# jbirky/alabi

Hardware: AMD Instinct MI355X
Metric: surrogate_mcmc_samples_per_sec (higher is better)
Workload: dtype f64

## Files before the change

alabi_amd/_lib.py:

```python
from __future__ import annotations

import ctypes as C
import os
import subprocess

_HERE = os.path.dirname(os.path.abspath(__file__))
CSRC = os.path.join(_HERE, "csrc")
LIB_PATH = os.path.join(CSRC, "libalabi_hip.so")

OK, NOT_PD, BAD_ARG, HIP_ERROR, NOT_COMPUTED, TIMEOUT = 0, 1, 2, 3, 4, 5
UTILITY_CODES = {"bape": 0, "agp": 1, "jones": 2}
KERNEL_CODES = {"ExpSquaredKernel": 0, "Matern32Kernel": 1, "Matern52Kernel": 2, "RationalQuadraticKernel": 3}
MAX_DIM = 64

_vp, _i, _ll, _d = C.c_void_p, C.c_int, C.c_longlong, C.c_double
_ull = C.c_ulonglong
_pd = C.POINTER(C.c_double)
_pi = C.POINTER(C.c_int)
_pll = C.POINTER(C.c_longlong)

SIGNATURES = {
    "alabi_abi_version": (_i, []),
    "alabi_status_string": (C.c_char_p, [_i]),
    "alabi_last_error": (C.c_char_p, []),
# ... 35 lines not shown
    "alabi_ens_set_logp_affine": (_i, [_vp, _d, _d]),
    "alabi_ens_set_normal_prior": (_i, [_vp, _pd, _pd]),
    "alabi_ens_set_logp_map": (_i, [_vp, _i]),
    "alabi_ens_surrogate": (_i, [_vp, _vp, _i, _vp, _vp]),
    "alabi_ens_propose": (_i, [_vp, _vp, _i, _i, _i, _vp, _vp, _vp]),
    "alabi_ens_accept": (_i, [_vp, _vp, _vp, _i, _i, _vp, _vp, _vp, _vp]),
    "alabi_ens_set_moves": (_i, [_vp, _i, _pi, _pd, _pd, _pd]),
    "alabi_ens_set_stream": (_i, [_vp, _i]),
    "alabi_ens_last_path": (_i, [_vp, _pi]),
    "alabi_ens_stream_variant": (_i, [_vp, _pi]),
    "alabi_ens_pair_stats": (_i, [_vp, _pll, _i]),
    "alabi_ens_pair_stats2": (_i, [_vp, _pll, _i]),
    "alabi_ens_group_plan": (_i, [_vp, _pi]),
    "alabi_ens_lnprob": (_i, [_vp, _vp, _vp, _vp]),
    "alabi_ens_run": (_i, [_vp, _vp, _vp, _ll, _ll, _i, _d, _vp, _vp, _vp, _vp]),
    "alabi_chain_autocorr": (_i, [_vp, _ll, _i, _i, _vp, _vp]),
    "alabi_ens_draw": (_i, [_vp, _ll, _i, _d, _vp]),
    "alabi_ens_half_step": (_i, [_vp, _vp, _vp, _i, _i, _i, _i, _vp, _vp]),
    "alabi_dist_unique_id": (_i, [_vp]),
    "alabi_dist_comm_create": (_i, [_vp, _i, _i, C.POINTER(_vp)]),
    "alabi_dist_comm_create_callback": (_i, [_vp, _vp, _i, _i, C.POINTER(_vp)]),
    "alabi_dist_comm_destroy": (_i, [_vp]),
    "alabi_dist_comm_stats": (_i, [_vp, _pll]),
    "alabi_ens_run_sharded": (_i, [_vp, _vp, _vp, _vp, _ll, _ll, _i, _d, _vp, _vp, _vp, _vp]),
    "alabi_ens_step_lists": (_i, [_vp, _i, _vp, _pi, _vp]),
    "alabi_ens_step_with_randoms": (_i, [_vp, _vp, _vp, _vp, _i, _vp, _vp, _vp, _d, _vp, _vp]),
    "alabi_ens_export_draws": (_i, [_vp, _ll, _d, _vp, _pi, _vp, _vp, _vp, _vp, _vp, _vp]),
    "alabi_ens_export_move_draws": (_i, [_vp, _vp, _vp, _vp, _vp]),
    "alabi_ens_step_with_randoms_de": (_i, [_vp, _vp, _vp, _vp, _i, _vp, _vp, _vp, _vp, _vp, _vp]),
    "alabi_ens_export_snooker_draws": (_i, [_vp, _vp, _vp]),
# ... 101 lines not shown
```

alabi_amd/csrc/api.hip:

```cpp
#include <atomic>
#include <cmath>
#include <cstdlib>
#include <mutex>
#include <new>
#include <vector>

#include "gp_device.hpp"

namespace alabi {
thread_local std::string g_last_error;

static inline hipStream_t as_stream(void* s) { return reinterpret_cast<hipStream_t>(s); }

__global__ void __launch_bounds__(256)
copy_factor_kernel(const double* __restrict__ L, int ld, int N, double* __restrict__ out) {
    size_t e = (size_t)blockIdx.x * 256 + threadIdx.x;
    if (e >= (size_t)N * N) return;
    int r = (int)(e / N), c = (int)(e % N);
    out[e] = (c <= r) ? L[(size_t)r * ld + c] : 0.0;
}

namespace {
struct CachedBuf { void* p; size_t bytes; };
std::mutex g_cache_mu;
// ... 540 lines not shown
    const size_t n = (size_t)e->chunk_cap * WT;
    DrawBuffers& b = e->draws;
    hipError_t err = alloc_draws(b, n);
    if (err == hipSuccess) err = hipMalloc(&e->run_state, 4 * sizeof(long long));
    if (err == hipSuccess) err = hipMalloc(&e->consts, 5 * ALABI_MAX_DIM * sizeof(double));
    {
        int dev = 0, n_cu = 0;
        const char* env = getenv("ALABI_ENS_STREAM");
        if (hipGetDevice(&dev) == hipSuccess &&
            hipDeviceGetAttribute(&n_cu, hipDeviceAttributeMultiprocessorCount, dev) == hipSuccess &&
            n_ensembles <= n_cu && !(env && env[0] == '0')) {
            int G = n_cu / n_ensembles;
            if (G > (W + 1) / 2) G = (W + 1) / 2;
            e->stream_grid = G;
            const size_t hist_words = ((size_t)e->chunk_cap + 1) * WT * (d + 2);
            if (err == hipSuccess) err = hipMalloc(&e->hist, hist_words * sizeof(unsigned long long));
            if (err == hipSuccess) err = hipMalloc(&e->err, sizeof(int));
            e->stream_ok = (err == hipSuccess) ? 1 : 0;
        }
    }
    if (err != hipSuccess) {
        alabi_ens_destroy(e);
        return hip_fail(err, "hipMalloc(ensemble buffers)", __FILE__, __LINE__);
    }
    *out = e;
    return ALABI_OK;
}

int alabi_ens_destroy(alabi_ens* e) {
    if (!e) return ALABI_OK;
    if (e->graph_exec) (void)hipGraphExecDestroy(e->graph_exec);
    free_draws(e->draws);
    free_draws(e->draws2);
    free_move_buffers(e->mv);
    if (e->side_stream) (void)hipStreamDestroy(e->side_stream);
    if (e->ev_free) (void)hipEventDestroy(e->ev_free);
    if (e->ev_drawn) (void)hipEventDestroy(e->ev_drawn);
    if (e->run_state) (void)hipFree(e->run_state);
    if (e->consts) (void)hipFree(e->consts);
    if (e->hist) (void)hipFree(e->hist);
    if (e->part) (void)hipFree(e->part);
    if (e->cand) (void)hipFree(e->cand);
    if (e->err) (void)hipFree(e->err);
    ens_pair_release(e);
    delete e;
    return ALABI_OK;
}

int alabi_ens_set_normal_prior(alabi_ens* e, const double* mean, const double* std) {
    if (!e || !mean || !std) return ALABI_BAD_ARGUMENT;
    e->has_prior = 0; e->prior_const = 0.0;
    for (int k = 0; k < ALABI_MAX_DIM; ++k) { e->prior_mean[k] = 0.0; e->prior_istd[k] = 0.0; }
    for (int k = 0; k < e->d; ++k) {
        if (std::isfinite(mean[k]) && std::isfinite(std[k]) && std[k] > 0.0) {
            e->prior_mean[k] = mean[k];
            e->prior_istd[k] = 1.0 / std[k];
            e->prior_const += -std::log(std[k]) - 0.9189385332046727;
            e->has_prior = 1;
// ... 32 lines not shown
        if (kind[k] == 0) { if (!(p0[k] > 1.0) || !std::isfinite(p0[k])) return ALABI_BAD_ARGUMENT; }
        else if (kind[k] == 1) { if (!std::isfinite(p0[k]) || !std::isfinite(p1[k])) return ALABI_BAD_ARGUMENT; de = true; }
        else if (kind[k] == 2) { if (!std::isfinite(p0[k])) return ALABI_BAD_ARGUMENT; snooker = true; }
        else return ALABI_BAD_ARGUMENT;
        mt.kind[k] = kind[k]; mt.cum[k] = cum[k]; mt.p0[k] = p0[k]; mt.p1[k] = p1[k];
    }
    if (n > 0 && !(prev > 0.0)) return ALABI_BAD_ARGUMENT;
    if (de && e->W < 4) return ALABI_BAD_ARGUMENT;
    if (snooker && e->W < 6) return ALABI_BAD_ARGUMENT;
    if (n > 0) { const int st = ensure_move_buffers(e, snooker); if (st != ALABI_OK) return st; }
    mt.n = n;
    e->moves = mt;
    e->has_de = de || snooker;
    e->has_snooker = snooker;
    e->drawn_n = 0;
    e->settings_gen++;
    if (e->graph_exec) { (void)hipGraphExecDestroy(e->graph_exec); e->graph_exec = nullptr; }
    return ALABI_OK;
}

int alabi_ens_set_stream(alabi_ens* e, int enabled) {
    if (!e) return ALABI_BAD_ARGUMENT;
    if (enabled && !(e->hist && e->err)) return ALABI_BAD_ARGUMENT;
    e->stream_ok = enabled ? 1 : 0;
    e->settings_gen++;
    return ALABI_OK;
}

int alabi_ens_stream_variant(alabi_ens* e, int* variant) {
    if (!e || !variant) return ALABI_BAD_ARGUMENT;
// ... 106 lines not shown
    const int n0 = h.n0, n1 = e->W - n0;
    const size_t WT = (size_t)e->W * e->E;
    for (int t = 0; t < n; ++t) {
        h.rec = offset_draws(e->draws, (size_t)t * WT);
        h.cw2 = e->has_de ? e->mv.cw2 + (size_t)t * WT : nullptr;
        h.cw3 = e->has_snooker ? e->mv.cw3 + (size_t)t * WT : nullptr;
        h.local_t = t; h.part_begin = 0;
        h.split = 0;
        if ((st = launch_ens_half_args(e, h, n0, s)) != ALABI_OK) return st;
        h.split = 1;
        if ((st = launch_ens_half_args(e, h, n1, s)) != ALABI_OK) return st;
    }
    return launch_ens_advance(e, n, s);
}

int alabi_ens_run(alabi_ens* e, double* coords, double* logp, long long step0, long long nsteps, int thin_by,
                  double a, double* chain, double* chain_logp, long long* n_accept, void* stream) {
    if (!e || !coords || !logp || nsteps < 0 || thin_by < 1 || !(a > 1.0)) return ALABI_BAD_ARGUMENT;
    if (!e->gp->computed || !e->gp->has_alpha) return ALABI_NOT_COMPUTED;
    if (nsteps == 0) return ALABI_OK;
    hipStream_t s = as_stream(stream);
    int st;
    if ((st = sync_consts(e, s)) != ALABI_OK) return st;
    e->last_path = 0;
    const char* genv = getenv("ALABI_ENS_GROUP");
    const bool group_off = genv && genv[0] == '0', group_pref = genv && genv[0] == '1';
    const bool can_stream = ens_stream_fits(e);
    const bool crowded = can_stream && e->stream_grid > 0 && ((e->W + 1) / 2 + e->stream_grid - 1) / e->stream_grid >= 4;
    const bool use_group = !e->has_de && e->stream_ok && s != nullptr && !group_off && (group_pref || !can_stream || crowded) && ens_group_fits(e) &&
                           ens_group_buffers(e, s);
    if (!e->has_de && e->stream_ok && s != nullptr && (can_stream || use_group)) {
        e->last_path = use_group ? 3 : 1;
        const int need = (int)(nsteps < e->chunk_cap ? nsteps : e->chunk_cap);
        const int clean_rows = e->hist_clean;
        e->hist_clean = 0;
        const bool use_pair = !use_group && can_stream && ens_pair_ready(e);
        e->last_variant = use_pair ? 1 : 0;
        const size_t WTs = (size_t)e->W * e->E;
        if (use_pair) {
            double* sv = e->pair_save;
            ALABI_HIP_CHECK(hipMemcpyAsync(sv, coords, WTs * e->d * sizeof(double), hipMemcpyDeviceToDevice, s));
            ALABI_HIP_CHECK(hipMemcpyAsync(sv + WTs * e->d, logp, WTs * sizeof(double), hipMemcpyDeviceToDevice, s));
            if (n_accept) ALABI_HIP_CHECK(hipMemcpyAsync(sv + WTs * (e->d + 1), n_accept, WTs * sizeof(long long), hipMemcpyDeviceToDevice, s));
        }
        if (use_group && (st = set_run_state(e, step0, 0, s)) != ALABI_OK) return st;
        ALABI_HIP_CHECK(hipMemsetAsync(e->err, 0, sizeof(int), s));
        long long remaining = nsteps;
        const bool two_sets = !use_group && nsteps > e->chunk_cap && ens_draw_ahead_ready(e);
        bool ahead_issued = false;
        while (remaining > 0) {
            const int K = (int)(remaining < e->chunk_cap ? remaining : e->chunk_cap);
            const long long done = nsteps - remaining;
            if (use_group) {
                if ((st = launch_ens_draw(e, K, a, s)) != ALABI_OK) return st;
                if ((st = launch_ens_group(e, coords, logp, K, thin_by, chain, chain_logp, n_accept, s)) != ALABI_OK) return st;
                if ((st = launch_ens_advance(e, K, s)) != ALABI_OK) return st;
            } else {
                const bool odd = two_sets && ((done / e->chunk_cap) & 1);
                const bool ahead = two_sets && remaining > K;
                const DrawBuffers& cur = odd ? e->draws2 : e->draws;
                if (ahead_issued) ALABI_HIP_CHECK(hipStreamWaitEvent(s, e->ev_drawn, 0));
                else if ((st = launch_ens_draw_at(e, cur, K, a, false, step0 + done, s)) != ALABI_OK) return st;
                ahead_issued = false;
                if (ahead) ALABI_HIP_CHECK(hipEventRecord(e->ev_free, s));
                const int fill_rows = (done == 0 && clean_rows < need) ? need : 0;
                if ((st = use_pair ? launch_ens_pair_kernel(e, cur, coords, logp, K, done == 0, fill_rows, s)
                                   : launch_ens_stream_kernel(e, cur, coords, logp, K, done == 0, fill_rows, s)) != ALABI_OK)
                    return st;
                if (ahead) {
                    const long long rem2 = remaining - K;
                    const int K2 = (int)(rem2 < e->chunk_cap ? rem2 : e->chunk_cap);
                    ALABI_HIP_CHECK(hipStreamWaitEvent(e->side_stream, e->ev_free, 0));
                    if ((st = launch_ens_draw_at(e, odd ? e->draws : e->draws2, K2, a, false, step0 + done + K, e->side_stream)) != ALABI_OK)
                        return st;
                    ALABI_HIP_CHECK(hipEventRecord(e->ev_drawn, e->side_stream));
                    ahead_issued = true;
                }
                if ((st = launch_ens_stream_epilogue(e, coords, logp, K, thin_by, chain, chain_logp, n_accept, step0 + done + K, done, s)) != ALABI_OK)
                    return st;
            }
            remaining -= K;
        }
        int flag = 0;
        ALABI_HIP_CHECK(hipMemcpyAsync(&flag, e->err, sizeof(int), hipMemcpyDeviceToHost, s));
        ALABI_HIP_CHECK(hipStreamSynchronize(s));
        e->hist_clean = (!use_group && !flag) ? (clean_rows > need ? clean_rows : need) : 0;
        if (flag && use_pair) {
            const double* sv = e->pair_save;
            ALABI_HIP_CHECK(hipMemcpyAsync(coords, sv, WTs * e->d * sizeof(double), hipMemcpyDeviceToDevice, s));
            ALABI_HIP_CHECK(hipMemcpyAsync(logp, sv + WTs * e->d, WTs * sizeof(double), hipMemcpyDeviceToDevice, s));
            if (n_accept) ALABI_HIP_CHECK(hipMemcpyAsync(n_accept, sv + WTs * (e->d + 1), WTs * sizeof(long long), hipMemcpyDeviceToDevice, s));
            e->pair_state = -1;
            return alabi_ens_run(e, coords, logp, step0, nsteps, thin_by, a, chain, chain_logp, n_accept, stream);
        }
        return flag ? ALABI_TIMEOUT : ALABI_OK;
    }
    if ((st = set_run_state(e, step0, 0, s)) != ALABI_OK) return st;
    HalfArgs h = base_args(e, coords, logp);
    h.chain = chain; h.chain_logp = chain_logp; h.n_accept = n_accept; h.thin_by = thin_by;

    const char* env = getenv("ALABI_ENS_GRAPH");
    const bool want_graph = (s != nullptr) && !(env && env[0] == '0');
    int gsteps = e->chunk_cap < 256 ? e->chunk_cap : 256;
    if (const char* gs = getenv("ALABI_ENS_GRAPH_STEPS")) {
        int v = atoi(gs);
        if (v > 0 && v <= e->chunk_cap) gsteps = v;
// ... 210 lines not shown
```

alabi_amd/csrc/common.hpp:

```cpp
#pragma once
#include <hip/hip_runtime.h>
#include <cstdint>
#include <cstdio>
#include <cstring>
#include <string>
#include <vector>

#include "../../include/alabi_hip.h"
#include "chol_tasks.hpp"

#define ALABI_BLK 64

namespace alabi {

extern thread_local std::string g_last_error;

inline int hip_fail(hipError_t e, const char* what, const char* file, int line) {
    char buf[512];
    snprintf(buf, sizeof(buf), "%s failed at %s:%d: %s", what, file, line, hipGetErrorString(e));
    g_last_error = buf;
    return ALABI_HIP_ERROR;
}

#define ALABI_HIP_CHECK(expr)                                                    \
// ... 116 lines not shown
    long long consts_gen = -1;
    int chunk_cap = 0;
    int drawn_n = 0;
    alabi::DrawBuffers draws{};
    hipGraphExec_t graph_exec = nullptr;
    struct GraphKey {
        void *coords, *logp, *chain, *chain_logp, *n_accept;
        int thin_by, nsteps;
        double a;
        long long gp_gen;
    } graph_key{};
    int graph_steps = 0;
    long long* run_state = nullptr;
    unsigned long long* hist = nullptr;
    int* err = nullptr;
    alabi::DrawBuffers draws2{};
    hipStream_t side_stream = nullptr;
    hipEvent_t ev_free = nullptr, ev_drawn = nullptr;
    int draws2_state = 0;
    int hist_clean = 0;
    int stream_grid = 0;
    int last_path = 0;
    int stream_ok = 0;
    unsigned long long* prop = nullptr;
    double* pair_save = nullptr;
#define ALABI_PAIR_STATS_WORDS 16
    unsigned long long* pair_stats = nullptr;
    int pair_state = 0;
    int last_variant = 0;
    unsigned long long* part = nullptr;
    size_t part_words = 0;
    unsigned long long* cand = nullptr;
    size_t cand_words = 0;
    long long settings_gen = 0;
    long long serial = 0;
    int group_plan[8] = {0};
    alabi::MoveTable moves{};
    bool has_de = false, has_snooker = false;
    alabi::MoveBuffers mv{};
};
// ... 78 lines not shown
                    const double* u_acc, double a, hipStream_t s);
int launch_ens_prep_de(alabi_ens* e, const int* order, int n0, const int* j1, const int* j2, const double* gamma,
                       const double* u_acc, hipStream_t s);
int launch_ens_prep_snooker(alabi_ens* e, const int* order, int n0, const int* j1, const int* j2, const int* j3, double gamma,
                            const double* u_acc, hipStream_t s);
int launch_ens_half_args(alabi_ens* e, const HalfArgs& args, int nblocks, hipStream_t s);
int launch_ens_lnprob(alabi_ens* e, const double* coords, int nwalkers, double* logp, int gate_box, hipStream_t s);
int launch_ens_propose(alabi_ens* e, const HalfArgs& args, int nblocks, int gate_box, double* q, double* like, hipStream_t s);
int launch_ens_accept(alabi_ens* e, const HalfArgs& args, int count, const double* q, const double* lp_new, hipStream_t s);
int launch_ens_advance(alabi_ens* e, long long n, hipStream_t s);
int ens_sync_consts(alabi_ens* e, hipStream_t s);
int alabi_ens_half_step_hist(alabi_ens* e, const double* coords, const double* logp, int t, int split, int part_begin, int part_end,
                             const double* shist, double* out, hipStream_t s);
bool ens_stream_fits(const alabi_ens* e);
int ens_stream_ppt(const alabi_ens* e);
int launch_ens_stream_kernel(alabi_ens* e, const DrawBuffers& rec, double* coords, double* logp, int K, bool first, int fill_rows, hipStream_t s);
int launch_ens_hist_fill(unsigned long long* rows, size_t words, hipStream_t s);
int launch_ens_stream_prologue(alabi_ens* e, double* coords, double* logp, bool first, int fill_rows, hipStream_t s);
int launch_ens_stream_epilogue(alabi_ens* e, double* coords, double* logp, int K, int thin_by, double* chain, double* chain_logp,
                               long long* n_accept, long long step_next, long long done0, hipStream_t s);
int launch_ens_hist_prologue(alabi_ens* e, double* coords, double* logp, int K, bool fill, hipStream_t s);
int launch_ens_hist_epilogue(alabi_ens* e, double* coords, double* logp, int K, int thin_by, double* chain, double* chain_logp,
                             long long* n_accept, hipStream_t s);
bool ens_pair_ready(alabi_ens* e);
void ens_pair_release(alabi_ens* e);
int launch_ens_pair_kernel(alabi_ens* e, const DrawBuffers& rec, double* coords, double* logp, int K, bool first, int fill_rows, hipStream_t s);
bool ens_group_fits(const alabi_ens* e);
bool ens_group_buffers(alabi_ens* e, hipStream_t s);
int launch_ens_group(alabi_ens* e, double* coords, double* logp, int K, int thin_by, double* chain, double* chain_logp,
                     long long* n_accept, hipStream_t s);
}
```

alabi_amd/csrc/ens_pair.hip:

```cpp
#include <cstdlib>
#include "ens_stream.hpp"

namespace alabi {

struct PairArgs {
    StreamArgs s;
    unsigned long long* prop;
    unsigned long long* stats;
};

#ifdef ALABI_PAIR_PROF
__device__ long long g_pair_prof[26];
#define ALABI_PAIR_PUB_MASK ((1 << 19) - 1)
__device__ long long g_pair_pub[2][ALABI_PAIR_PUB_MASK + 1];
__device__ inline void pair_pub_stamp(int which, size_t row_index) {
    __hip_atomic_store(&g_pair_pub[which][row_index & ALABI_PAIR_PUB_MASK], wall_clock64(), __ATOMIC_RELAXED, __HIP_MEMORY_SCOPE_AGENT);
}
__device__ inline long long pair_pub_age(int which, size_t row_index, long long now) {
    const long long dt = now - __hip_atomic_load(&g_pair_pub[which][row_index & ALABI_PAIR_PUB_MASK], __ATOMIC_RELAXED, __HIP_MEMORY_SCOPE_AGENT);
    return (dt > 0 && dt < 100000) ? dt : -1;
}
#endif

template <int D, int PPT, int TMAX, bool GENERIC>
// ... 257 lines not shown
#endif

bool ens_pair_ready(alabi_ens* e) {
    if (e->pair_state < 0) return false;
    if (e->pair_state == 0) {
        e->pair_state = -1;
        const char* env = getenv("ALABI_ENS_PAIR");
        if (env && env[0] == '0') return false;
        int dev = 0, n_cu = 0;
        if (hipGetDevice(&dev) != hipSuccess || hipDeviceGetAttribute(&n_cu, hipDeviceAttributeMultiprocessorCount, dev) != hipSuccess) return false;
        const long long wgs = 2LL * ((e->W + 1) / 2) * e->E;
        if (e->d < 1 || wgs > n_cu) return false;
        const size_t WT = (size_t)e->W * e->E, row = e->d + 2;
        const size_t words = ((size_t)e->chunk_cap + 1) * WT * row;
        if (hipMalloc(&e->prop, words * sizeof(unsigned long long)) != hipSuccess) { (void)hipGetLastError(); e->prop = nullptr; return false; }
        if (hipMalloc(&e->pair_save, (WT * (e->d + 1)) * sizeof(double) + WT * sizeof(long long)) != hipSuccess) {
            (void)hipGetLastError(); (void)hipFree(e->prop); e->prop = nullptr; e->pair_save = nullptr; return false;
        }
        e->pair_state = 1;
    }
    return true;
}

void ens_pair_release(alabi_ens* e) {
    if (e->prop) (void)hipFree(e->prop);
    if (e->pair_save) (void)hipFree(e->pair_save);
    if (e->pair_stats) (void)hipFree(e->pair_stats);
    e->prop = nullptr; e->pair_save = nullptr; e->pair_stats = nullptr;
}

int launch_ens_pair_kernel(alabi_ens* e, const DrawBuffers& rec, double* coords, double* logp, int K, bool first, int fill_rows,
                           hipStream_t s) {
    const int n0 = (e->W + 1) / 2;
    const int WT = e->W * e->E, row = e->d + 2;
    int st = launch_ens_stream_prologue(e, coords, logp, first, fill_rows, s);
    if (st != ALABI_OK) return st;
    if ((st = launch_ens_hist_fill(e->prop + (size_t)WT * row, (size_t)K * WT * row, s)) != ALABI_OK) return st;
    PairArgs a{};
    a.s = ens_stream_args(e, rec, K);
    a.prop = e->prop; a.stats = e->pair_stats;
    e->last_path = 1;
    st = ens_stream_dispatch(e, [&](auto D, auto PPT, auto TMAX, auto GENERIC) {
        hipLaunchKernelGGL((ens_pair_kernel<D(), PPT(), TMAX(), GENERIC()>), dim3(2 * n0, e->E), dim3(TMAX()), 0, s, a);
    });
    if (st != ALABI_OK) return st;
    ALABI_LAUNCH_CHECK();
    return ALABI_OK;
}

}
```

alabi_amd/csrc/ens_stream.hip:

```cpp
#include <cstdlib>
#include "ens_stream.hpp"

namespace alabi {

#ifdef ALABI_STREAM_PROF
__device__ long long g_stream_prof[16];
#endif

template <int D, int PPT, int TMAX, bool GENERIC>
__global__ void __launch_bounds__(TMAX)
ens_stream_kernel(StreamArgs p) {
    __shared__ __attribute__((aligned(16))) double scratch[2][16];
    __shared__ unsigned long long rec_s[4][4];
    __shared__ __attribute__((aligned(16))) double qs_s[2][ALABI_MAX_DIM];
    __shared__ double consts_s[6][ALABI_MAX_DIM];
    __shared__ int abort_s;
    static_assert(D < ALABI_MAX_DIM && TMAX >= 192 && TMAX % 64 == 0, "ens_stream_kernel: shape");
    constexpr int TC = TMAX - 128, nwc = TC >> 6;
    const int tid = threadIdx.x, lane = tid & 63;
    const int wv = __builtin_amdgcn_readfirstlane(tid >> 6);
    const bool comm = wv == 0, service = wv == nwc + 1, compute = !comm && !service;
    const int b = blockIdx.x, e = blockIdx.y, E = gridDim.y;
    const int WT = p.W * E, row = p.d + 2;
#ifdef ALABI_STREAM_PROF
// ... 133 lines not shown
}

__global__ void __launch_bounds__(256)
ens_hist_copy_kernel(double* __restrict__ coords, double* __restrict__ logp, unsigned long long* __restrict__ hist_row,
                     int WT, int d, int to_hist) {
    const int i = blockIdx.x * 256 + threadIdx.x, row = d + 2;
    if (i >= WT * row) return;
    const int w = i / row, k = i % row;
    if (k > d) { if (to_hist) hist_row[i] = 0ull; return; }
    double* src = (k < d) ? coords + (size_t)w * d + k : logp + w;
    if (to_hist) hist_row[i] = (unsigned long long)__double_as_longlong(*src);
    else *src = __longlong_as_double((long long)hist_row[i]);
}

__global__ void __launch_bounds__(256)
ens_hist_chain_kernel(const unsigned long long* __restrict__ hist, int K, int WT, int d, int thin_by,
                      const long long* __restrict__ run_state, const int* __restrict__ err, double* __restrict__ chain,
                      double* __restrict__ chain_logp, unsigned long long* __restrict__ n_accept) {
    if (*err) return;
    const int row = d + 2;
    const size_t n = (size_t)K * WT * row;
    const long long done0 = run_state[1];
    for (size_t i = (size_t)blockIdx.x * 256 + threadIdx.x; i < n; i += (size_t)gridDim.x * 256) {
        const int k = (int)(i % row);
        const size_t vw = i / row;
        const int w = (int)(vw % WT), v = (int)(vw / WT) + 1;
        const unsigned long long word = hist[(size_t)WT * row + i];
        if (k == d + 1) { if (word == 1ull && n_accept) atomicAdd(n_accept + w, 1ull); continue; }
        const long long done = done0 + v;
        if (done % thin_by != 0) continue;
        const size_t slot = (size_t)(done / thin_by - 1);
        if (k < d) { if (chain) chain[(slot * WT + w) * d + k] = __longlong_as_double((long long)word); }
        else if (chain_logp) chain_logp[slot * WT + w] = __longlong_as_double((long long)word);
    }
}

#define ALABI_EPI_VG 16
__global__ void __launch_bounds__(256)
ens_hist_epilogue_kernel(unsigned long long* __restrict__ hist, int K, int WT, int d, int thin_by, long long step_next, long long done0,
                         const int* __restrict__ err, double* __restrict__ coords, double* __restrict__ logp, double* __restrict__ chain,
                         double* __restrict__ chain_logp, unsigned long long* __restrict__ n_accept, long long* __restrict__ run_state) {
    const int k = threadIdx.x, row = d + 2;
    const int w = blockIdx.x * blockDim.y + threadIdx.y;
    if (blockIdx.x == 0 && blockIdx.y == 0 && threadIdx.x == 0 && threadIdx.y == 0) { run_state[0] = step_next; run_state[1] = done0 + K; }
    if (*err) return;
    if (k >= row || w >= WT) return;
    const int v0 = 1 + blockIdx.y * ALABI_EPI_VG;
    const int v1 = (v0 + ALABI_EPI_VG - 1 < K) ? v0 + ALABI_EPI_VG - 1 : K;
    long long slot = (done0 + v0) / thin_by;
    int phase = (int)((done0 + v0) % thin_by);
    const size_t vstride = (size_t)WT * row;
    unsigned long long* hp = hist + (size_t)v0 * vstride + (size_t)w * row + k;
    unsigned long long nacc = 0;
    for (int v = v0; v <= v1; v += 4, hp += 4 * vstride) {
        unsigned long long word[4];
#pragma unroll
        for (int j = 0; j < 4; ++j) word[j] = (v + j <= v1) ? hp[j * vstride] : 0ull;
#pragma unroll
        for (int j = 0; j < 4; ++j) {
            if (v + j > v1) break;
            hp[j * vstride] = ALABI_HIST_EMPTY;
            if (k == d + 1) nacc += (word[j] == 1ull) ? 1ull : 0ull;
            else {
                const double val = __longlong_as_double((long long)word[j]);
                if (phase == 0) {
                    const size_t sw = (size_t)(slot - 1) * WT + w;
                    if (k < d) { if (chain) chain[sw * d + k] = val; }
                    else if (chain_logp) chain_logp[sw] = val;
                }
                if (v + j == K) {
                    hist[(size_t)w * row + k] = word[j];
                    if (k < d) coords[(size_t)w * d + k] = val; else logp[w] = val;
                }
            }
            if (++phase == thin_by) { phase = 0; ++slot; }
        }
    }
    if (k == d + 1 && n_accept && nacc) atomicAdd(n_accept + w, nacc);
}

int ens_stream_ppt(const alabi_ens* e) {
    const int T = e->threads, half = e->gp->Npad / 2, db = dim_bucket(e->d);
    if (e->d > 61 || db < 0) return 0;
    if (e->ymap != 0) return 0;
    const int ppt = (half + T - 1) / T;
    return db <= ens_stream_max_db(T, ppt, e->gp->kf.type != 0) ? ppt : 0;
}
// ... 14 lines not shown
    hipLaunchKernelGGL(ens_hist_copy_kernel, dim3((WT * row + 255) / 256), dim3(256), 0, s, coords, logp,
                       e->hist + (size_t)K * WT * row, WT, e->d, 0);
    if (chain || chain_logp || n_accept)
        hipLaunchKernelGGL(ens_hist_chain_kernel, dim3(2048), dim3(256), 0, s, e->hist, K, WT, e->d, thin_by, e->run_state,
                           e->err, chain, chain_logp, reinterpret_cast<unsigned long long*>(n_accept));
    ALABI_LAUNCH_CHECK();
    return ALABI_OK;
}

int launch_ens_hist_fill(unsigned long long* rows, size_t words, hipStream_t s) {
    hipLaunchKernelGGL(ens_hist_fill_kernel, dim3(1024), dim3(256), 0, s, rows, words);
    ALABI_LAUNCH_CHECK();
    return ALABI_OK;
}

int launch_ens_stream_prologue(alabi_ens* e, double* coords, double* logp, bool first, int fill_rows, hipStream_t s) {
    const int WT = e->W * e->E, row = e->d + 2;
    if (fill_rows > 0) hipLaunchKernelGGL(ens_hist_fill_kernel, dim3(1024), dim3(256), 0, s, e->hist + (size_t)WT * row, (size_t)fill_rows * WT * row);
    if (first) hipLaunchKernelGGL(ens_hist_copy_kernel, dim3((WT * row + 255) / 256), dim3(256), 0, s, coords, logp, e->hist, WT, e->d, 1);
    ALABI_LAUNCH_CHECK();
    return ALABI_OK;
}

StreamArgs ens_stream_args(alabi_ens* e, const DrawBuffers& rec, int K) {
    alabi_gp* gp = e->gp;
    StreamArgs a{};
    a.hist = e->hist; a.err = e->err; a.rec = rec; a.consts = e->consts;
    const bool se = gp->kf.type == 0;
    a.Xt = se ? gp->Xc : gp->Xt; a.alpha = se ? gp->ens_h : gp->alpha; a.centre = gp->xa_centre;
    a.K = K; a.W = e->W; a.n0 = (e->W + 1) / 2; a.d = e->d; a.Npad = gp->Npad; a.spin_limit = 1 << 20;
    if (const char* env = getenv("ALABI_ENS_SPIN_LIMIT")) { const int v = atoi(env); if (v > 0) a.spin_limit = v; }
    a.amp = e->lp_scale * exp(gp->log_amp); a.mean = fma(e->lp_scale, gp->mean, e->lp_shift); a.kf = gp->kf;
    a.has_prior = e->has_prior; a.prior_const = e->prior_const;
    return a;
}

int launch_ens_stream_kernel(alabi_ens* e, const DrawBuffers& rec, double* coords, double* logp, int K, bool first, int fill_rows,
                             hipStream_t s) {
    int st = launch_ens_stream_prologue(e, coords, logp, first, fill_rows, s);
    if (st != ALABI_OK) return st;
    const StreamArgs a = ens_stream_args(e, rec, K);
    e->last_path = 1;
    st = ens_stream_dispatch(e, [&](auto D, auto PPT, auto TMAX, auto GENERIC) {
        hipLaunchKernelGGL((ens_stream_kernel<D(), PPT(), TMAX(), GENERIC()>), dim3(e->stream_grid, e->E), dim3(TMAX()), 0, s, a);
    });
    if (st != ALABI_OK) return st;
    ALABI_LAUNCH_CHECK();
    return ALABI_OK;
}

int launch_ens_stream_epilogue(alabi_ens* e, double* coords, double* logp, int K, int thin_by, double* chain, double* chain_logp,
                               long long* n_accept, long long step_next, long long done0, hipStream_t s) {
    const int WT = e->W * e->E, row = e->d + 2;
    int rp = 16;
    while (rp < row) rp <<= 1;
    const int wb = 256 / rp;
    hipLaunchKernelGGL(ens_hist_epilogue_kernel, dim3((WT + wb - 1) / wb, (K + ALABI_EPI_VG - 1) / ALABI_EPI_VG), dim3(rp, wb), 0, s,
                       e->hist, K, WT, e->d, thin_by, step_next, done0, e->err, coords, logp, chain, chain_logp,
                       reinterpret_cast<unsigned long long*>(n_accept), e->run_state);
    ALABI_LAUNCH_CHECK();
    return ALABI_OK;
}

}
```

alabi_amd/sampler.py:

```python
from __future__ import annotations

import ctypes as C
import time

import numpy as np
import torch

from . import _lib
from .gp import HipGP, _dev, _to_dev
from .mcmc_utils import integrated_time
from .moves import parse_moves

__all__ = ["EnsembleSampler", "State"]


class State:
    def __init__(self, coords, log_prob=None):
        self.coords = coords
        self.log_prob = log_prob
        self.blobs = None
        self.random_state = None

    def __iter__(self):
        return iter((self.coords, self.log_prob, self.random_state))
# ... 250 lines not shown
                return State(self._coords.cpu().numpy(), self._logp.cpu().numpy())
        nstore = nsteps // thin_by if store else 0
        dev = self._coords.device
        chain = torch.empty((nstore, self.total_walkers, self.ndim), dtype=torch.float64, device=dev) if nstore else None
        chain_lp = torch.empty((nstore, self.total_walkers), dtype=torch.float64, device=dev) if nstore else None
        t0 = time.perf_counter()
        if self.generic:
            self._run_generic(nsteps, thin_by, chain, chain_lp)
            self.last_path = "host-callback"
            self.last_run_seconds = time.perf_counter() - t0
            self.iteration += nsteps
            self._rng_step += nsteps
            if nstore:
                self._chains.append(chain); self._chain_lps.append(chain_lp); self._thins.append(thin_by)
            return State(self._coords.cpu().numpy(), self._logp.cpu().numpy())
        backup = (self._coords.clone(), self._logp.clone(), self._naccept.clone())
        self._stream.wait_stream(torch.cuda.current_stream())

        def _run():
            with torch.cuda.stream(self._stream):
                return _lib.lib().alabi_ens_run(self._ens, _lib.ptr(self._coords), _lib.ptr(self._logp), self._rng_step,
                                                nsteps, thin_by, self.a, _lib.ptr(chain), _lib.ptr(chain_lp),
                                                _lib.ptr(self._naccept), C.c_void_p(self._stream.cuda_stream))

        st = _run()
        if st == _lib.TIMEOUT:
            self._stream.synchronize()
            self._coords.copy_(backup[0]); self._logp.copy_(backup[1]); self._naccept.copy_(backup[2])
            _lib.check(_lib.lib().alabi_ens_set_stream(self._ens, 0), "alabi_ens_set_stream")
            self.stream_fallbacks = getattr(self, "stream_fallbacks", 0) + 1
            st = _run()
        _lib.check(st, "alabi_ens_run")
        path = C.c_int(0)
        _lib.lib().alabi_ens_last_path(self._ens, C.byref(path))
        self.last_path = {1: "stream", 3: "group"}.get(path.value, "launch-per-half-step")
        self.last_stream_kernel = {1: "ens_stream_kernel", 3: "ens_group_kernel"}.get(path.value)
        variant = C.c_int(0)
        _lib.lib().alabi_ens_stream_variant(self._ens, C.byref(variant))
        self.last_stream_variant = {0: "single", 1: "pair"}[variant.value] if path.value == 1 else None
        self.group_plan = None
        if path.value == 3:
            plan = (C.c_int * 8)()
            _lib.lib().alabi_ens_group_plan(self._ens, plan)
            self.group_plan = dict(zip(("Q", "G", "NG", "RT", "tpm", "ltw", "KS", "lds_bytes"), (int(v) for v in plan)))
        self._stream.synchronize()
        torch.cuda.current_stream().wait_stream(self._stream)
        self.last_run_seconds = time.perf_counter() - t0
        self.iteration += nsteps
        self._rng_step += nsteps
        if nstore:
            self._chains.append(chain)
            self._chain_lps.append(chain_lp)
            self._thins.append(thin_by)
        return State(self._coords.cpu().numpy(), self._logp.cpu().numpy())

    def reset(self):
        self._chains, self._chain_lps, self._thins = [], [], []
        self._naccept.zero_()
        self.iteration = 0
        self._tau_memo = None

    def get_chain_device(self, discard=0, thin=1, flat=False, log_prob=False):
        src = self._chain_lps if log_prob else self._chains
        if not src:
            raise AttributeError("you must run the sampler with 'store == True' before accessing the results")
        v = src[0] if len(src) == 1 else torch.cat(src, dim=0)
        v = v[discard + thin - 1::thin]
        if flat:
# ... 28 lines not shown
```

include/alabi_hip.h:

```cpp
#ifndef ALABI_HIP_H
#define ALABI_HIP_H

#ifdef __cplusplus
extern "C" {
#endif

#define ALABI_OK 0
#define ALABI_NOT_POSITIVE_DEFINITE 1
#define ALABI_BAD_ARGUMENT 2
#define ALABI_HIP_ERROR 3
#define ALABI_NOT_COMPUTED 4
#define ALABI_TIMEOUT 5

#define ALABI_UTILITY_BAPE 0
#define ALABI_UTILITY_AGP 1
#define ALABI_UTILITY_JONES 2

#define ALABI_MAX_DIM 64

typedef struct alabi_gp alabi_gp;
typedef struct alabi_ens alabi_ens;
typedef struct alabi_ns alabi_ns;
typedef struct alabi_kde alabi_kde;

// ... 79 lines not shown

int alabi_ens_set_stream(alabi_ens* ens, int enabled);
int alabi_ens_last_path(alabi_ens* ens, int* path );
int alabi_ens_stream_variant(alabi_ens* ens, int* variant );
int alabi_ens_pair_stats(alabi_ens* ens, long long* out , int reset);
int alabi_ens_pair_stats2(alabi_ens* ens, long long* out , int enable);
int alabi_ens_group_plan(alabi_ens* ens, int* out );

int alabi_ens_lnprob(alabi_ens* ens, const double* coords, double* logp, void* stream);

int alabi_ens_surrogate(alabi_ens* ens, const double* points, int M, double* like, void* stream);

int alabi_ens_run(alabi_ens* ens, double* coords, double* logp, long long step0,
                  long long nsteps, int thin_by, double a, double* chain, double* chain_logp,
                  long long* n_accept, void* stream);

int alabi_chain_autocorr(const double* chain, long long n_t, int n_w, int n_d, double* acf_mean, void* stream);

int alabi_ens_draw(alabi_ens* ens, long long step0, int nsteps, double a, void* stream);
int alabi_ens_half_step(alabi_ens* ens, double* coords, double* logp, int t, int split,
                        int part_begin, int part_end, long long* n_accept, void* stream);
int alabi_ens_propose(alabi_ens* ens, const double* coords, int t, int split, int gate_box,
                      double* q, double* like, void* stream);
int alabi_ens_accept(alabi_ens* ens, double* coords, double* logp, int t, int split,
                     const double* q, const double* lp_new, long long* n_accept, void* stream);
typedef struct alabi_comm alabi_comm;
typedef int (*alabi_allgather_fn)(const double* send_dev, double* recv_dev, long long count_per_rank, void* user, void* stream);
int alabi_dist_unique_id(void* id_out );
int alabi_dist_comm_create(const void* id , int rank, int nranks, alabi_comm** out);
int alabi_dist_comm_create_callback(alabi_allgather_fn fn, void* user, int rank, int nranks, alabi_comm** out);
// ... 74 lines not shown
```

Before: 97.07 million.

## Prefetch next call's draws, fuse state backup, return final state in one readback

Each ensemble run now issues the random draws for the next call's first chunk on the side stream after the last chunk and reuses them on a matching next call. A fused prologue kernel replaces the Python-side clone backup, the separate memsets and the history copy. The epilogue writes the final coords and logp next to the error flag so a single pinned readback returns them, and the host no longer makes separate .cpu() copies. The proposal buffer is cleaned in the epilogue so it needs no refill on the next call. This adds cross-call state (ahead validity, generation counters) that can go stale if settings change.

```diff
diff --git a/alabi_amd/_lib.py b/alabi_amd/_lib.py
--- a/alabi_amd/_lib.py
+++ b/alabi_amd/_lib.py
@@ -73,6 +73,9 @@
     "alabi_ens_group_plan": (_i, [_vp, _pi]),
     "alabi_ens_lnprob": (_i, [_vp, _vp, _vp, _vp]),
     "alabi_ens_run": (_i, [_vp, _vp, _vp, _ll, _ll, _i, _d, _vp, _vp, _vp, _vp]),
+    "alabi_ens_last_state": (_i, [_vp, _vp, _vp]),
+    "alabi_ens_restore": (_i, [_vp, _vp, _vp, _vp, _vp]),
+    "alabi_ens_boundary_stats": (_i, [_vp, _pll]),
     "alabi_chain_autocorr": (_i, [_vp, _ll, _i, _i, _vp, _vp]),
     "alabi_ens_draw": (_i, [_vp, _ll, _i, _d, _vp]),
     "alabi_ens_half_step": (_i, [_vp, _vp, _vp, _i, _i, _i, _i, _vp, _vp]),
diff --git a/alabi_amd/csrc/api.hip b/alabi_amd/csrc/api.hip
--- a/alabi_amd/csrc/api.hip
+++ b/alabi_amd/csrc/api.hip
@@ -1,6 +1,7 @@
 #include <atomic>
 #include <cmath>
 #include <cstdlib>
+#include <cstring>
 #include <mutex>
 #include <new>
 #include <vector>
@@ -578,8 +579,13 @@
             if (G > (W + 1) / 2) G = (W + 1) / 2;
             e->stream_grid = G;
             const size_t hist_words = ((size_t)e->chunk_cap + 1) * WT * (d + 2);
+            const size_t state_words = 1 + (size_t)WT * (d + 1);
             if (err == hipSuccess) err = hipMalloc(&e->hist, hist_words * sizeof(unsigned long long));
-            if (err == hipSuccess) err = hipMalloc(&e->err, sizeof(int));
+            if (err == hipSuccess) err = hipMalloc(&e->state_dev, state_words * sizeof(unsigned long long));
+            if (err == hipSuccess) err = hipMemset(e->state_dev, 0, state_words * sizeof(unsigned long long));
+            if (err == hipSuccess) err = hipHostMalloc(reinterpret_cast<void**>(&e->state_host), state_words * sizeof(unsigned long long), hipHostMallocDefault);
+            if (err == hipSuccess) err = hipMalloc(&e->save, (size_t)WT * (d + 1) * sizeof(double) + (size_t)WT * sizeof(long long));
+            if (err == hipSuccess) e->err = reinterpret_cast<int*>(e->state_dev);
             e->stream_ok = (err == hipSuccess) ? 1 : 0;
         }
     }
@@ -594,6 +600,7 @@
 int alabi_ens_destroy(alabi_ens* e) {
     if (!e) return ALABI_OK;
     if (e->graph_exec) (void)hipGraphExecDestroy(e->graph_exec);
+    if (e->side_stream) (void)hipStreamSynchronize(e->side_stream);
     free_draws(e->draws);
     free_draws(e->draws2);
     free_move_buffers(e->mv);
@@ -605,7 +612,9 @@
     if (e->hist) (void)hipFree(e->hist);
     if (e->part) (void)hipFree(e->part);
     if (e->cand) (void)hipFree(e->cand);
-    if (e->err) (void)hipFree(e->err);
+    if (e->state_dev) (void)hipFree(e->state_dev);
+    if (e->state_host) (void)hipHostFree(e->state_host);
+    if (e->save) (void)hipFree(e->save);
     ens_pair_release(e);
     delete e;
     return ALABI_OK;
@@ -668,6 +677,8 @@
     e->has_de = de || snooker;
     e->has_snooker = snooker;
     e->drawn_n = 0;
+    e->ahead_valid = false;
+    e->moves_gen++;
     e->settings_gen++;
     if (e->graph_exec) { (void)hipGraphExecDestroy(e->graph_exec); e->graph_exec = nullptr; }
     return ALABI_OK;
@@ -804,6 +815,37 @@
     return launch_ens_advance(e, n, s);
 }
 
+static int ens_restore(alabi_ens* e, double* coords, double* logp, long long* n_accept, hipStream_t s) {
+    if (!e->save || !e->save_valid) return ALABI_NOT_COMPUTED;
+    const size_t WT = (size_t)e->W * e->E;
+    const double* sv = e->save;
+    ALABI_HIP_CHECK(hipMemcpyAsync(coords, sv, WT * e->d * sizeof(double), hipMemcpyDeviceToDevice, s));
+    ALABI_HIP_CHECK(hipMemcpyAsync(logp, sv + WT * e->d, WT * sizeof(double), hipMemcpyDeviceToDevice, s));
+    if (n_accept && e->save_accept)
+        ALABI_HIP_CHECK(hipMemcpyAsync(n_accept, sv + WT * (e->d + 1), WT * sizeof(long long), hipMemcpyDeviceToDevice, s));
+    return ALABI_OK;
+}
+
+int alabi_ens_restore(alabi_ens* e, double* coords, double* logp, long long* n_accept, void* stream) {
+    if (!e || !coords || !logp) return ALABI_BAD_ARGUMENT;
+    return ens_restore(e, coords, logp, n_accept, as_stream(stream));
+}
+
+int alabi_ens_last_state(alabi_ens* e, double* coords_out, double* logp_out) {
+    if (!e || !coords_out || !logp_out) return ALABI_BAD_ARGUMENT;
+    if (!e->last_state_ok || !e->state_host) return ALABI_NOT_COMPUTED;
+    const size_t WT = (size_t)e->W * e->E;
+    memcpy(coords_out, e->state_host + 1, WT * e->d * sizeof(double));
+    memcpy(logp_out, e->state_host + 1 + WT * e->d, WT * sizeof(double));
+    return ALABI_OK;
+}
+
+int alabi_ens_boundary_stats(alabi_ens* e, long long* out) {
+    if (!e || !out) return ALABI_BAD_ARGUMENT;
+    for (int i = 0; i < 4; ++i) out[i] = e->boundary_stats[i];
+    return ALABI_OK;
+}
+
 int alabi_ens_run(alabi_ens* e, double* coords, double* logp, long long step0, long long nsteps, int thin_by,
                   double a, double* chain, double* chain_logp, long long* n_accept, void* stream) {
     if (!e || !coords || !logp || nsteps < 0 || thin_by < 1 || !(a > 1.0)) return ALABI_BAD_ARGUMENT;
@@ -813,6 +855,7 @@
     int st;
     if ((st = sync_consts(e, s)) != ALABI_OK) return st;
     e->last_path = 0;
+    e->last_state_ok = false;
     const char* genv = getenv("ALABI_ENS_GROUP");
     const bool group_off = genv && genv[0] == '0', group_pref = genv && genv[0] == '1';
     const bool can_stream = ens_stream_fits(e);
@@ -826,18 +869,22 @@
         e->hist_clean = 0;
         const bool use_pair = !use_group && can_stream && ens_pair_ready(e);
         e->last_variant = use_pair ? 1 : 0;
-        const size_t WTs = (size_t)e->W * e->E;
-        if (use_pair) {
-            double* sv = e->pair_save;
-            ALABI_HIP_CHECK(hipMemcpyAsync(sv, coords, WTs * e->d * sizeof(double), hipMemcpyDeviceToDevice, s));
-            ALABI_HIP_CHECK(hipMemcpyAsync(sv + WTs * e->d, logp, WTs * sizeof(double), hipMemcpyDeviceToDevice, s));
-            if (n_accept) ALABI_HIP_CHECK(hipMemcpyAsync(sv + WTs * (e->d + 1), n_accept, WTs * sizeof(long long), hipMemcpyDeviceToDevice, s));
+        const int prop_clean_rows = use_pair ? e->prop_clean : 0;
+        if (use_pair) e->prop_clean = 0;
+        if (use_group && (st = set_run_state(e, step0, 0, s)) != ALABI_OK) return st;
+        const bool two_sets = !use_group && ens_draw_ahead_ready(e);
+        bool ahead_issued = false;
+        if (!use_group) {
+            const bool hit = two_sets && e->ahead_valid && e->ahead_step == step0 && e->ahead_a == a && e->ahead_moves_gen == e->moves_gen &&
+                             need <= e->ahead_n;
+            if (e->ahead_pending) ALABI_HIP_CHECK(hipStreamWaitEvent(s, e->ev_drawn, 0));
+            e->ahead_pending = false; e->ahead_valid = false;
+            e->draw_set = hit ? 1 : 0;
+            e->boundary_stats[hit ? 0 : 1]++;
+            if (!hit && (st = launch_ens_draw_at(e, e->draws, need, a, false, step0, s)) != ALABI_OK) return st;
         }
-        if (use_group && (st = set_run_state(e, step0, 0, s)) != ALABI_OK) return st;
-        ALABI_HIP_CHECK(hipMemsetAsync(e->err, 0, sizeof(int), s));
+        if ((st = launch_ens_call_prologue(e, coords, logp, n_accept, !use_group, s)) != ALABI_OK) return st;
         long long remaining = nsteps;
-        const bool two_sets = !use_group && nsteps > e->chunk_cap && ens_draw_ahead_ready(e);
-        bool ahead_issued = false;
         while (remaining > 0) {
             const int K = (int)(remaining < e->chunk_cap ? remaining : e->chunk_cap);
             const long long done = nsteps - remaining;
@@ -846,40 +893,52 @@
                 if ((st = launch_ens_group(e, coords, logp, K, thin_by, chain, chain_logp, n_accept, s)) != ALABI_OK) return st;
                 if ((st = launch_ens_advance(e, K, s)) != ALABI_OK) return st;
             } else {
-                const bool odd = two_sets && ((done / e->chunk_cap) & 1);
-                const bool ahead = two_sets && remaining > K;
-                const DrawBuffers& cur = odd ? e->draws2 : e->draws;
+                const bool last = remaining == K;
+                const bool ahead = two_sets;
+                const DrawBuffers& cur = e->draw_set ? e->draws2 : e->draws;
                 if (ahead_issued) ALABI_HIP_CHECK(hipStreamWaitEvent(s, e->ev_drawn, 0));
-                else if ((st = launch_ens_draw_at(e, cur, K, a, false, step0 + done, s)) != ALABI_OK) return st;
+                else if (done > 0 && (st = launch_ens_draw_at(e, cur, K, a, false, step0 + done, s)) != ALABI_OK) return st;
                 ahead_issued = false;
-                if (ahead) ALABI_HIP_CHECK(hipEventRecord(e->ev_free, s));
+                if (ahead && !last) ALABI_HIP_CHECK(hipEventRecord(e->ev_free, s));
                 const int fill_rows = (done == 0 && clean_rows < need) ? need : 0;
-                if ((st = use_pair ? launch_ens_pair_kernel(e, cur, coords, logp, K, done == 0, fill_rows, s)
-                                   : launch_ens_stream_kernel(e, cur, coords, logp, K, done == 0, fill_rows, s)) != ALABI_OK)
+                const int prop_fill_rows = (done == 0 && prop_clean_rows < need) ? need : 0;
+                if ((st = use_pair ? launch_ens_pair_kernel(e, cur, K, fill_rows, prop_fill_rows, s)
+                                   : launch_ens_stream_kernel(e, cur, K, fill_rows, s)) != ALABI_OK)
                     return st;
+                if (ahead && last) ALABI_HIP_CHECK(hipEventRecord(e->ev_free, s));
                 if (ahead) {
                     const long long rem2 = remaining - K;
-                    const int K2 = (int)(rem2 < e->chunk_cap ? rem2 : e->chunk_cap);
+                    const int K2 = last ? e->chunk_cap : (int)(rem2 < e->chunk_cap ? rem2 : e->chunk_cap);
                     ALABI_HIP_CHECK(hipStreamWaitEvent(e->side_stream, e->ev_free, 0));
-                    if ((st = launch_ens_draw_at(e, odd ? e->draws : e->draws2, K2, a, false, step0 + done + K, e->side_stream)) != ALABI_OK)
+                    if ((st = launch_ens_draw_at(e, (last || e->draw_set == 0) ? e->draws2 : e->draws, K2, a, false, step0 + done + K,
+                                                 e->side_stream)) != ALABI_OK)
                         return st;
                     ALABI_HIP_CHECK(hipEventRecord(e->ev_drawn, e->side_stream));
-                    ahead_issued = true;
+                    if (last) {
+                        e->ahead_pending = true; e->ahead_valid = true;
+                        e->ahead_step = step0 + nsteps; e->ahead_a = a; e->ahead_moves_gen = e->moves_gen; e->ahead_n = K2;
+                    } else {
+                        ahead_issued = true;
+                    }
                 }
-                if ((st = launch_ens_stream_epilogue(e, coords, logp, K, thin_by, chain, chain_logp, n_accept, step0 + done + K, done, s)) != ALABI_OK)
+                if ((st = launch_ens_stream_epilogue(e, coords, logp, K, thin_by, chain, chain_logp, n_accept, step0 + done + K, done,
+                                                     use_pair, last, s)) != ALABI_OK)
                     return st;
+                if (two_sets) e->draw_set ^= 1;
             }
             remaining -= K;
         }
-        int flag = 0;
-        ALABI_HIP_CHECK(hipMemcpyAsync(&flag, e->err, sizeof(int), hipMemcpyDeviceToHost, s));
+        const size_t WTs = (size_t)e->W * e->E;
+        const size_t back = use_group ? sizeof(unsigned long long) : (1 + WTs * (e->d + 1)) * sizeof(unsigned long long);
+        ALABI_HIP_CHECK(hipMemcpyAsync(e->state_host, e->state_dev, back, hipMemcpyDeviceToHost, s));
         ALABI_HIP_CHECK(hipStreamSynchronize(s));
+        const int flag = *reinterpret_cast<const int*>(e->state_host);
         e->hist_clean = (!use_group && !flag) ? (clean_rows > need ? clean_rows : need) : 0;
+        if (use_pair) e->prop_clean = !flag ? (prop_clean_rows > need ? prop_clean_rows : need) : 0;
+        e->last_state_ok = !use_group && !flag;
+        if (flag) e->ahead_valid = false;
         if (flag && use_pair) {
-            const double* sv = e->pair_save;
-            ALABI_HIP_CHECK(hipMemcpyAsync(coords, sv, WTs * e->d * sizeof(double), hipMemcpyDeviceToDevice, s));
-            ALABI_HIP_CHECK(hipMemcpyAsync(logp, sv + WTs * e->d, WTs * sizeof(double), hipMemcpyDeviceToDevice, s));
-            if (n_accept) ALABI_HIP_CHECK(hipMemcpyAsync(n_accept, sv + WTs * (e->d + 1), WTs * sizeof(long long), hipMemcpyDeviceToDevice, s));
+            if ((st = ens_restore(e, coords, logp, n_accept, s)) != ALABI_OK) return st;
             e->pair_state = -1;
             return alabi_ens_run(e, coords, logp, step0, nsteps, thin_by, a, chain, chain_logp, n_accept, stream);
         }
diff --git a/alabi_amd/csrc/common.hpp b/alabi_amd/csrc/common.hpp
--- a/alabi_amd/csrc/common.hpp
+++ b/alabi_amd/csrc/common.hpp
@@ -154,16 +154,28 @@
     long long* run_state = nullptr;
     unsigned long long* hist = nullptr;
     int* err = nullptr;
+    unsigned long long* state_dev = nullptr;
+    unsigned long long* state_host = nullptr;
+    bool last_state_ok = false;
+    double* save = nullptr;
+    bool save_valid = false, save_accept = false;
     alabi::DrawBuffers draws2{};
     hipStream_t side_stream = nullptr;
     hipEvent_t ev_free = nullptr, ev_drawn = nullptr;
     int draws2_state = 0;
+    int draw_set = 0;
+    bool ahead_valid = false, ahead_pending = false;
+    long long ahead_step = 0, ahead_moves_gen = 0;
+    double ahead_a = 0.0;
+    int ahead_n = 0;
+    long long moves_gen = 0;
+    long long boundary_stats[4] = {0, 0, 0, 0};
     int hist_clean = 0;
+    int prop_clean = 0;
     int stream_grid = 0;
     int last_path = 0;
     int stream_ok = 0;
     unsigned long long* prop = nullptr;
-    double* pair_save = nullptr;
 #define ALABI_PAIR_STATS_WORDS 16
     unsigned long long* pair_stats = nullptr;
     int pair_state = 0;
@@ -272,17 +284,17 @@
                              const double* shist, double* out, hipStream_t s);
 bool ens_stream_fits(const alabi_ens* e);
 int ens_stream_ppt(const alabi_ens* e);
-int launch_ens_stream_kernel(alabi_ens* e, const DrawBuffers& rec, double* coords, double* logp, int K, bool first, int fill_rows, hipStream_t s);
+int launch_ens_stream_kernel(alabi_ens* e, const DrawBuffers& rec, int K, int fill_rows, hipStream_t s);
 int launch_ens_hist_fill(unsigned long long* rows, size_t words, hipStream_t s);
-int launch_ens_stream_prologue(alabi_ens* e, double* coords, double* logp, bool first, int fill_rows, hipStream_t s);
+int launch_ens_call_prologue(alabi_ens* e, const double* coords, const double* logp, const long long* n_accept, bool row0, hipStream_t s);
 int launch_ens_stream_epilogue(alabi_ens* e, double* coords, double* logp, int K, int thin_by, double* chain, double* chain_logp,
-                               long long* n_accept, long long step_next, long long done0, hipStream_t s);
+                               long long* n_accept, long long step_next, long long done0, bool clean_prop, bool last, hipStream_t s);
 int launch_ens_hist_prologue(alabi_ens* e, double* coords, double* logp, int K, bool fill, hipStream_t s);
 int launch_ens_hist_epilogue(alabi_ens* e, double* coords, double* logp, int K, int thin_by, double* chain, double* chain_logp,
                              long long* n_accept, hipStream_t s);
 bool ens_pair_ready(alabi_ens* e);
 void ens_pair_release(alabi_ens* e);
-int launch_ens_pair_kernel(alabi_ens* e, const DrawBuffers& rec, double* coords, double* logp, int K, bool first, int fill_rows, hipStream_t s);
+int launch_ens_pair_kernel(alabi_ens* e, const DrawBuffers& rec, int K, int fill_rows, int prop_fill_rows, hipStream_t s);
 bool ens_group_fits(const alabi_ens* e);
 bool ens_group_buffers(alabi_ens* e, hipStream_t s);
 int launch_ens_group(alabi_ens* e, double* coords, double* logp, int K, int thin_by, double* chain, double* chain_logp,
diff --git a/alabi_amd/csrc/ens_pair.hip b/alabi_amd/csrc/ens_pair.hip
--- a/alabi_amd/csrc/ens_pair.hip
+++ b/alabi_amd/csrc/ens_pair.hip
@@ -295,9 +295,7 @@
         const size_t WT = (size_t)e->W * e->E, row = e->d + 2;
         const size_t words = ((size_t)e->chunk_cap + 1) * WT * row;
         if (hipMalloc(&e->prop, words * sizeof(unsigned long long)) != hipSuccess) { (void)hipGetLastError(); e->prop = nullptr; return false; }
-        if (hipMalloc(&e->pair_save, (WT * (e->d + 1)) * sizeof(double) + WT * sizeof(long long)) != hipSuccess) {
-            (void)hipGetLastError(); (void)hipFree(e->prop); e->prop = nullptr; e->pair_save = nullptr; return false;
-        }
+        e->prop_clean = 0;
         e->pair_state = 1;
     }
     return true;
@@ -305,18 +303,22 @@
 
 void ens_pair_release(alabi_ens* e) {
     if (e->prop) (void)hipFree(e->prop);
-    if (e->pair_save) (void)hipFree(e->pair_save);
     if (e->pair_stats) (void)hipFree(e->pair_stats);
-    e->prop = nullptr; e->pair_save = nullptr; e->pair_stats = nullptr;
-}
-
-int launch_ens_pair_kernel(alabi_ens* e, const DrawBuffers& rec, double* coords, double* logp, int K, bool first, int fill_rows,
-                           hipStream_t s) {
+    e->prop = nullptr; e->pair_stats = nullptr;
+}
+
+int launch_ens_pair_kernel(alabi_ens* e, const DrawBuffers& rec, int K, int fill_rows, int prop_fill_rows, hipStream_t s) {
     const int n0 = (e->W + 1) / 2;
-    const int WT = e->W * e->E, row = e->d + 2;
-    int st = launch_ens_stream_prologue(e, coords, logp, first, fill_rows, s);
-    if (st != ALABI_OK) return st;
-    if ((st = launch_ens_hist_fill(e->prop + (size_t)WT * row, (size_t)K * WT * row, s)) != ALABI_OK) return st;
+    const size_t WT = (size_t)e->W * e->E, row = e->d + 2;
+    int st;
+    if (fill_rows > 0) {
+        if ((st = launch_ens_hist_fill(e->hist + WT * row, (size_t)fill_rows * WT * row, s)) != ALABI_OK) return st;
+        e->boundary_stats[3]++;
+    }
+    if (prop_fill_rows > 0) {
+        if ((st = launch_ens_hist_fill(e->prop + WT * row, (size_t)prop_fill_rows * WT * row, s)) != ALABI_OK) return st;
+        e->boundary_stats[2]++;
+    }
     PairArgs a{};
     a.s = ens_stream_args(e, rec, K);
     a.prop = e->prop; a.stats = e->pair_stats;
diff --git a/alabi_amd/csrc/ens_stream.hip b/alabi_amd/csrc/ens_stream.hip
--- a/alabi_amd/csrc/ens_stream.hip
+++ b/alabi_amd/csrc/ens_stream.hip
@@ -171,6 +171,23 @@
 }
 
 __global__ void __launch_bounds__(256)
+ens_call_prologue_kernel(const double* __restrict__ coords, const double* __restrict__ logp, const long long* __restrict__ n_accept,
+                         double* __restrict__ save, unsigned long long* __restrict__ hist_row0, int* __restrict__ err, int WT, int d) {
+    const int i = blockIdx.x * 256 + threadIdx.x, row = d + 2;
+    if (i == 0) *err = 0;
+    if (i >= WT * row) return;
+    const int w = i / row, k = i % row;
+    if (k > d) {
+        if (hist_row0) hist_row0[i] = 0ull;
+        if (n_accept) reinterpret_cast<long long*>(save + (size_t)WT * (d + 1))[w] = n_accept[w];
+        return;
+    }
+    const double v = (k < d) ? coords[(size_t)w * d + k] : logp[w];
+    save[(k < d) ? (size_t)w * d + k : (size_t)WT * d + w] = v;
+    if (hist_row0) hist_row0[i] = (unsigned long long)__double_as_longlong(v);
+}
+
+__global__ void __launch_bounds__(256)
 ens_hist_chain_kernel(const unsigned long long* __restrict__ hist, int K, int WT, int d, int thin_by,
                       const long long* __restrict__ run_state, const int* __restrict__ err, double* __restrict__ chain,
                       double* __restrict__ chain_logp, unsigned long long* __restrict__ n_accept) {
@@ -196,7 +213,8 @@
 __global__ void __launch_bounds__(256)
 ens_hist_epilogue_kernel(unsigned long long* __restrict__ hist, int K, int WT, int d, int thin_by, long long step_next, long long done0,
                          const int* __restrict__ err, double* __restrict__ coords, double* __restrict__ logp, double* __restrict__ chain,
-                         double* __restrict__ chain_logp, unsigned long long* __restrict__ n_accept, long long* __restrict__ run_state) {
+                         double* __restrict__ chain_logp, unsigned long long* __restrict__ n_accept, long long* __restrict__ run_state,
+                         unsigned long long* __restrict__ prop, double* __restrict__ state_out) {
     const int k = threadIdx.x, row = d + 2;
     const int w = blockIdx.x * blockDim.y + threadIdx.y;
     if (blockIdx.x == 0 && blockIdx.y == 0 && threadIdx.x == 0 && threadIdx.y == 0) { run_state[0] = step_next; run_state[1] = done0 + K; }
@@ -207,7 +225,9 @@
     long long slot = (done0 + v0) / thin_by;
     int phase = (int)((done0 + v0) % thin_by);
     const size_t vstride = (size_t)WT * row;
-    unsigned long long* hp = hist + (size_t)v0 * vstride + (size_t)w * row + k;
+    const size_t first = (size_t)v0 * vstride + (size_t)w * row + k;
+    unsigned long long* hp = hist + first;
+    unsigned long long* pp = prop ? prop + first : nullptr;
     unsigned long long nacc = 0;
     for (int v = v0; v <= v1; v += 4, hp += 4 * vstride) {
         unsigned long long word[4];
@@ -217,6 +237,7 @@
         for (int j = 0; j < 4; ++j) {
             if (v + j > v1) break;
             hp[j * vstride] = ALABI_HIST_EMPTY;
+            if (pp) pp[(size_t)(v - v0 + j) * vstride] = ALABI_HIST_EMPTY;
             if (k == d + 1) nacc += (word[j] == 1ull) ? 1ull : 0ull;
             else {
                 const double val = __longlong_as_double((long long)word[j]);
@@ -228,6 +249,7 @@
                 if (v + j == K) {
                     hist[(size_t)w * row + k] = word[j];
                     if (k < d) coords[(size_t)w * d + k] = val; else logp[w] = val;
+                    if (state_out) state_out[(k < d) ? (size_t)w * d + k : (size_t)WT * d + w] = val;
                 }
             }
             if (++phase == thin_by) { phase = 0; ++slot; }
@@ -272,11 +294,12 @@
     return ALABI_OK;
 }
 
-int launch_ens_stream_prologue(alabi_ens* e, double* coords, double* logp, bool first, int fill_rows, hipStream_t s) {
+int launch_ens_call_prologue(alabi_ens* e, const double* coords, const double* logp, const long long* n_accept, bool row0, hipStream_t s) {
     const int WT = e->W * e->E, row = e->d + 2;
-    if (fill_rows > 0) hipLaunchKernelGGL(ens_hist_fill_kernel, dim3(1024), dim3(256), 0, s, e->hist + (size_t)WT * row, (size_t)fill_rows * WT * row);
-    if (first) hipLaunchKernelGGL(ens_hist_copy_kernel, dim3((WT * row + 255) / 256), dim3(256), 0, s, coords, logp, e->hist, WT, e->d, 1);
-    ALABI_LAUNCH_CHECK();
+    hipLaunchKernelGGL(ens_call_prologue_kernel, dim3((WT * row + 255) / 256), dim3(256), 0, s, coords, logp, n_accept, e->save,
+                       row0 ? e->hist : nullptr, e->err, WT, e->d);
+    ALABI_LAUNCH_CHECK();
+    e->save_valid = true; e->save_accept = n_accept != nullptr;
     return ALABI_OK;
 }
 
@@ -293,10 +316,13 @@
     return a;
 }
 
-int launch_ens_stream_kernel(alabi_ens* e, const DrawBuffers& rec, double* coords, double* logp, int K, bool first, int fill_rows,
-                             hipStream_t s) {
-    int st = launch_ens_stream_prologue(e, coords, logp, first, fill_rows, s);
-    if (st != ALABI_OK) return st;
+int launch_ens_stream_kernel(alabi_ens* e, const DrawBuffers& rec, int K, int fill_rows, hipStream_t s) {
+    int st;
+    if (fill_rows > 0) {
+        const size_t WT = (size_t)e->W * e->E, row = e->d + 2;
+        if ((st = launch_ens_hist_fill(e->hist + WT * row, (size_t)fill_rows * WT * row, s)) != ALABI_OK) return st;
+        e->boundary_stats[3]++;
+    }
     const StreamArgs a = ens_stream_args(e, rec, K);
     e->last_path = 1;
     st = ens_stream_dispatch(e, [&](auto D, auto PPT, auto TMAX, auto GENERIC) {
@@ -308,16 +334,17 @@
 }
 
 int launch_ens_stream_epilogue(alabi_ens* e, double* coords, double* logp, int K, int thin_by, double* chain, double* chain_logp,
-                               long long* n_accept, long long step_next, long long done0, hipStream_t s) {
+                               long long* n_accept, long long step_next, long long done0, bool clean_prop, bool last, hipStream_t s) {
     const int WT = e->W * e->E, row = e->d + 2;
     int rp = 16;
     while (rp < row) rp <<= 1;
     const int wb = 256 / rp;
     hipLaunchKernelGGL(ens_hist_epilogue_kernel, dim3((WT + wb - 1) / wb, (K + ALABI_EPI_VG - 1) / ALABI_EPI_VG), dim3(rp, wb), 0, s,
                        e->hist, K, WT, e->d, thin_by, step_next, done0, e->err, coords, logp, chain, chain_logp,
-                       reinterpret_cast<unsigned long long*>(n_accept), e->run_state);
-    ALABI_LAUNCH_CHECK();
-    return ALABI_OK;
-}
-
-}
+                       reinterpret_cast<unsigned long long*>(n_accept), e->run_state, clean_prop ? e->prop : nullptr,
+                       last ? reinterpret_cast<double*>(e->state_dev + 1) : nullptr);
+    ALABI_LAUNCH_CHECK();
+    return ALABI_OK;
+}
+
+}
diff --git a/alabi_amd/sampler.py b/alabi_amd/sampler.py
--- a/alabi_amd/sampler.py
+++ b/alabi_amd/sampler.py
@@ -288,7 +288,6 @@
             if nstore:
                 self._chains.append(chain); self._chain_lps.append(chain_lp); self._thins.append(thin_by)
             return State(self._coords.cpu().numpy(), self._logp.cpu().numpy())
-        backup = (self._coords.clone(), self._logp.clone(), self._naccept.clone())
         self._stream.wait_stream(torch.cuda.current_stream())
 
         def _run():
@@ -300,7 +299,8 @@
         st = _run()
         if st == _lib.TIMEOUT:
             self._stream.synchronize()
-            self._coords.copy_(backup[0]); self._logp.copy_(backup[1]); self._naccept.copy_(backup[2])
+            _lib.check(_lib.lib().alabi_ens_restore(self._ens, _lib.ptr(self._coords), _lib.ptr(self._logp), _lib.ptr(self._naccept),
+                                                    C.c_void_p(self._stream.cuda_stream)), "alabi_ens_restore")
             _lib.check(_lib.lib().alabi_ens_set_stream(self._ens, 0), "alabi_ens_set_stream")
             self.stream_fallbacks = getattr(self, "stream_fallbacks", 0) + 1
             st = _run()
@@ -326,6 +326,12 @@
             self._chains.append(chain)
             self._chain_lps.append(chain_lp)
             self._thins.append(thin_by)
+        if path.value == 1:
+            c = np.empty((self.total_walkers, self.ndim), dtype=np.float64)
+            lp = np.empty(self.total_walkers, dtype=np.float64)
+            _lib.check(_lib.lib().alabi_ens_last_state(self._ens, C.c_void_p(c.ctypes.data), C.c_void_p(lp.ctypes.data)),
+                       "alabi_ens_last_state")
+            return State(c, lp)
         return State(self._coords.cpu().numpy(), self._logp.cpu().numpy())
 
     def reset(self):
diff --git a/include/alabi_hip.h b/include/alabi_hip.h
--- a/include/alabi_hip.h
+++ b/include/alabi_hip.h
@@ -117,6 +117,9 @@
 int alabi_ens_run(alabi_ens* ens, double* coords, double* logp, long long step0,
                   long long nsteps, int thin_by, double a, double* chain, double* chain_logp,
                   long long* n_accept, void* stream);
+int alabi_ens_last_state(alabi_ens* ens, double* coords_out , double* logp_out );
+int alabi_ens_restore(alabi_ens* ens, double* coords, double* logp, long long* n_accept, void* stream);
+int alabi_ens_boundary_stats(alabi_ens* ens, long long* out );
 
 int alabi_chain_autocorr(const double* chain, long long n_t, int n_w, int n_d, double* acf_mean, void* stream);
 
```

Result: faster. 98.66 million (median of 6 runs) (+1.6%).
